# davrempe/humor

Hardware: AMD Instinct MI355X
Metric: fitting closure evaluations/s (stage-3 objective fwd+bwd), batch=32 seq=60 per GPU (higher is better)
Workload: dtype f32

## Files before the change

### humor_amd/_lib.py

```python
import ctypes as C
import os

_HERE = os.path.dirname(os.path.abspath(__file__))
DEFAULT_LIB = os.path.join(_HERE, 'csrc', 'libhumor_amd.so')

HA_OK = 0
ABI_VERSION = 7

c_float_p = C.POINTER(C.c_float)
c_int_p = C.POINTER(C.c_int32)


class MlpDesc(C.Structure):
    _fields_ = [('n_linear', C.c_int), ('in_dim', C.c_int), ('skip_dim', C.c_int), ('out_dims', C.c_int * 8),
                ('w', C.c_void_p * 8), ('b', C.c_void_p * 8), ('gn_gamma', C.c_void_p * 8), ('gn_beta', C.c_void_p * 8)]


FIT_NTERMS = 17


class GmmArgs(C.Structure):
    _fields_ = ([('B', C.c_int), ('K', C.c_int), ('D', C.c_int), ('nseg', C.c_int), ('seg', C.c_void_p * 4), ('seg_width', C.c_int * 4),
                 ('seg_stride', C.c_int * 4)] + [(n, C.c_void_p) for n in ('means', 'Linv', 'LinvT', 'cst', 'lp', 'gpart', 'nll', 'g_x')])

# ... 49 lines not shown
    'ha_device_arch': (C.c_int, [C.c_int, C.c_char_p, C.c_int]),
    'ha_tune_set': (C.c_int, [C.c_char_p, C.c_int]),
    'ha_debug_cu_poison': (C.c_int, [C.c_uint, C.POINTER(C.c_uint), C.c_void_p]),
    'ha_smpl_model_create': (C.c_int, [C.POINTER(C.c_void_p), C.c_int, C.c_int, C.c_int, C.c_int] + [C.c_void_p] * 6),
    'ha_smpl_model_destroy': (C.c_int, [C.c_void_p]),
    'ha_smpl_model_info': (C.c_int, [C.c_void_p, C.c_int, C.POINTER(C.c_int)]),
    'ha_smpl_model_define_subset': (C.c_int, [C.c_void_p, C.c_int, C.c_void_p, C.c_int]),
    'ha_smpl_forward': (C.c_int, [C.c_void_p, C.c_int, C.c_int, C.c_int] + [C.c_void_p] * 8 + [C.c_int, C.c_void_p]),
    'ha_smpl_workspace': (C.c_int, [C.c_void_p, C.c_int, C.c_int, C.POINTER(C.c_int64), C.POINTER(C.c_int64)]),
    'ha_smpl_backward': (C.c_int, [C.c_void_p, C.c_int, C.c_int, C.c_int] + [C.c_void_p] * 7 + [C.c_void_p]),
    'ha_smpl_forward_split': (C.c_int, [C.c_void_p, C.c_int, C.c_int, C.c_int] + [C.c_void_p] * 3 + [C.c_int] + [C.c_void_p] * 3),
    'ha_smpl_backward_split': (C.c_int, [C.c_void_p, C.c_int, C.c_int, C.c_int] + [C.c_void_p] * 2 + [C.c_int] + [C.c_void_p] * 6),
    'ha_smpl_forward_parts': (C.c_int, [C.c_void_p, C.c_int, C.c_int, C.c_int] + [C.c_void_p] * 3 + [C.c_int, C.c_void_p, C.c_int] + [C.c_void_p] * 3),
    'ha_smpl_backward_parts': (C.c_int, [C.c_void_p, C.c_int, C.c_int, C.c_int] + [C.c_void_p] * 3 + [C.c_int, C.c_int, C.c_void_p, C.c_int, C.c_int]
                               + [C.c_void_p] * 10),
    'ha_seq_sum_add': (C.c_int, [C.c_int, C.c_int, C.c_int] + [C.c_void_p] * 5),
    'ha_humor_rollout_backward_ex': (C.c_int, [C.c_void_p, C.c_int, C.c_int] + [C.c_void_p] * 8 + [C.c_void_p]),
    'ha_smpl_backward_dense_workspace': (C.c_int, [C.c_void_p, C.c_int, C.c_int, C.POINTER(C.c_int64)]),
    'ha_smpl_backward_dense': (C.c_int, [C.c_void_p, C.c_int, C.c_int] + [C.c_void_p] * 10 + [C.c_void_p]),
    'ha_lbs_skin': (C.c_int, [C.c_void_p, C.c_int] + [C.c_void_p] * 4 + [C.c_void_p]),
    'ha_rodrigues_fwd': (C.c_int, [C.c_int, C.c_void_p, C.c_void_p, C.c_void_p]),
    'ha_rodrigues_bwd': (C.c_int, [C.c_int, C.c_void_p, C.c_void_p, C.c_void_p, C.c_void_p]),
    'ha_rotmat_to_aa_fwd': (C.c_int, [C.c_int, C.c_void_p, C.c_void_p, C.c_void_p]),
    'ha_rotmat_to_aa_bwd': (C.c_int, [C.c_int, C.c_void_p, C.c_void_p, C.c_void_p, C.c_void_p]),
    'ha_rot6d_to_rotmat_fwd': (C.c_int, [C.c_int, C.c_void_p, C.c_void_p, C.c_void_p]),
    'ha_rot6d_to_rotmat_bwd': (C.c_int, [C.c_int, C.c_void_p, C.c_void_p, C.c_void_p, C.c_void_p]),
    'ha_rot9d_to_rotmat_fwd': (C.c_int, [C.c_int, C.c_void_p, C.c_void_p, C.c_void_p]),
    'ha_rot9d_to_rotmat_bwd': (C.c_int, [C.c_int, C.c_void_p, C.c_void_p, C.c_void_p, C.c_void_p]),
    'ha_humor_net_create': (C.c_int, [C.POINTER(C.c_void_p), C.c_int, C.POINTER(MlpDesc), C.POINTER(MlpDesc)]),
    'ha_humor_net_destroy': (C.c_int, [C.c_void_p]),
# ... 111 lines not shown
```

### humor_amd/csrc/smpl.hip

```cpp
#include <stdarg.h>
#include <string.h>
#include <algorithm>

#include <vector>

#include "smpl_model.h"
#ifndef HA_SIMT_EMU
#include "lane_reduce.h"
#endif

namespace ha {

static thread_local char g_err[512] = "";
void set_error(const char* fmt, ...) {
  va_list ap;
  va_start(ap, fmt);
  vsnprintf(g_err, sizeof(g_err), fmt, ap);
  va_end(ap);
}

}

namespace ha {
int g_skin_variant = -1;
int g_dense_gA_sparse = 2;
int g_dense_bwd_waves = 0;
extern int g_layer_finish, g_gemm_rm, g_rollout_groups, g_gemm_ks, g_gemm_fold, g_rollout_persist, g_rollout_persist_bwd, g_rollout_persist_inject, g_rollout_pipe, g_rollout_pipe_bwd;
extern unsigned g_cu_poison;
extern int g_loss_merge;
}
extern "C" int ha_tune_set(const char* key, int value) {
  HA_REQUIRE(key, "ha_tune_set: null key");
  if (strcmp(key, "skin_variant") == 0) { ha::g_skin_variant = value; return HA_OK; }
  if (strcmp(key, "dense_bwd_waves") == 0) { ha::g_dense_bwd_waves = value; return HA_OK; }
  if (strcmp(key, "dense_gA_sparse") == 0) { ha::g_dense_gA_sparse = value; return HA_OK; }
  if (strcmp(key, "layer_finish") == 0) { ha::g_layer_finish = value; return HA_OK; }
  if (strcmp(key, "gemm_rm") == 0) { ha::g_gemm_rm = value; return HA_OK; }
  if (strcmp(key, "rollout_groups") == 0) { ha::g_rollout_groups = value; return HA_OK; }
  if (strcmp(key, "gemm_ks") == 0) { ha::g_gemm_ks = value; return HA_OK; }
  if (strcmp(key, "gemm_fold") == 0) { ha::g_gemm_fold = value; return HA_OK; }
  if (strcmp(key, "rollout_persist") == 0) { ha::g_rollout_persist = value; return HA_OK; }
  if (strcmp(key, "rollout_persist_bwd") == 0) { ha::g_rollout_persist_bwd = value; return HA_OK; }
  if (strcmp(key, "rollout_pipe") == 0) { ha::g_rollout_pipe = value; return HA_OK; }
  if (strcmp(key, "rollout_pipe_bwd") == 0) { ha::g_rollout_pipe_bwd = value; return HA_OK; }
  if (strcmp(key, "loss_merge") == 0) { ha::g_loss_merge = value; return HA_OK; }
  if (strcmp(key, "rollout_persist_inject") == 0) { ha::g_rollout_persist_inject = value; return HA_OK; }
  if (strcmp(key, "cu_poison") == 0) { ha::g_cu_poison = (unsigned)value; return HA_OK; }
  ha::set_error("ha_tune_set: unknown key '%s'", key);
  return HA_ERR_INVALID_ARG;
}
extern "C" const char* ha_last_error(void) { return ha::g_err; }
extern "C" int ha_abi_version(void) { return 7; }
extern "C" int ha_device_arch(int device, char* buf, int buflen) {
  HA_REQUIRE(buf && buflen > 0, "ha_device_arch: null buffer");
  hipDeviceProp_t prop;
  HA_CHECK_HIP(hipGetDeviceProperties(&prop, device));
  snprintf(buf, buflen, "%s", prop.gcnArchName);
  return HA_OK;
}

namespace ha {

template <typename T>
static int upload(T** dst, const std::vector<T>& src) {
  *dst = nullptr;
  if (src.empty()) return HA_OK;
  HA_CHECK_HIP(hipMalloc((void**)dst, src.size() * sizeof(T)));
// ... 290 lines not shown
  const float* Jt; const float* Js; const int32_t* parents; const int32_t* jdepth;
  const int32_t* child_start; const int32_t* child_idx; const int32_t* anc; int nrounds;
  int J, NB, Kfull, Kfull_pad, kf4, depth;
  const float* Pd_v; const float* Pd_k; int Kp; const float* w; const int32_t* idx; const float* Wc;
  int nverts, nchunks, nnz;
  int N, n_active, Kc;
  const float* pose; const float* betas; const float* transl;
  float* verts; float* joints; float* A_out; float* coeffT; int Npad;
  int n_head, jstride;
  const float* g_verts; const float* g_joints;
  float* g_pose; float* g_betas; float* g_transl;
  const float* gA_in; const float* gco_part; int gco_ks, gco_rows, gco_ld; const float* gtl_part; int gtl_np;
  const float* pose_body; int betas_div; int gj_rows, gj_stride;
  float* g_body;
  const float* add_root; const float* add_body; const float* add_betas; const float* add_transl;
};

__device__ __forceinline__ const float* pose_of(const FrameParams& p, int f, int j, int J) {
  if (!p.pose_body) return p.pose + ((size_t)f * J + j) * 3;
  return j == 0 ? p.pose + (size_t)f * 3 : p.pose_body + ((size_t)f * (p.n_active - 1) + (j - 1)) * 3;
}
__device__ __forceinline__ const float* betas_of(const FrameParams& p, int f) {
  return p.betas + (size_t)(p.betas_div > 1 ? f / p.betas_div : f) * p.NB;
}

constexpr int FW = 4;

__device__ __forceinline__ void wave_sum16_all(float (&v)[16]) {
#ifdef HA_SIMT_EMU
#pragma unroll
  for (int i = 0; i < 16; ++i) {
// ... 183 lines not shown
  float* coeff = smem + wave * per_wave;
  float* Gs = coeff + p.kf4;
  int f = blockIdx.x * FW + wave;
  const bool valid = f < p.N;
  if (!valid) f = p.N - 1;

  SPT(0, 0);
  JointState s;
  joint_forward(p, f, lane, coeff, Gs, s);
  SPT(0, 1);

  float tl[3] = {0.f, 0.f, 0.f};
  if (p.transl) { tl[0] = p.transl[(size_t)f * 3]; tl[1] = p.transl[(size_t)f * 3 + 1]; tl[2] = p.transl[(size_t)f * 3 + 2]; }

  const bool isj = lane < p.J;
  float A[12];
  if (isj) {
    float gj[3];
    mat3_vec(s.G, s.Jr, gj);
#pragma unroll
    for (int i = 0; i < 9; ++i) A[i] = s.G[i];
#pragma unroll
    for (int c = 0; c < 3; ++c) A[9 + c] = s.G[9 + c] - gj[c];
#pragma unroll
    for (int i = 0; i < 12; ++i) Gs[lane * 12 + i] = A[i];
    if (valid) {
      if (p.joints) {
#pragma unroll
        for (int c = 0; c < 3; ++c) p.joints[((size_t)f * p.jstride + lane) * 3 + c] = s.G[9 + c] + tl[c];
      }
// ... 11 lines not shown
      v.x = 4 * q < p.kf4 ? coeff[4 * q] : 0.f;
      v.y = 4 * q + 1 < p.kf4 ? coeff[4 * q + 1] : 0.f;
      v.z = 4 * q + 2 < p.kf4 ? coeff[4 * q + 2] : 0.f;
      v.w = 4 * q + 3 < p.kf4 ? coeff[4 * q + 3] : 0.f;
      *reinterpret_cast<float4*>(p.coeffT + ((size_t)q * p.Npad + f) * 4) = v;
    }
  }
  if (p.verts) {
    for (int chunk = 0; chunk < p.nchunks; ++chunk) {
      float vp[3], T[12];
      SkinEntries sk;
      load_skin(p, chunk, lane, sk);
      SPT(0, 2);
      blend_vertex_block(p, chunk, wave, lane, smem, per_wave, smem + FW * per_wave, vp);
      SPT(0, 3);
      blend_transform(p, chunk, lane, sk, Gs, T);
      const int v = chunk * 64 + lane;
      if (valid && v < p.nverts) {
        float o[3];
        mat3_vec(T, vp, o);
        float* dst = v < p.n_head ? p.joints + ((size_t)f * p.jstride + p.J + v) * 3
                                  : p.verts + ((size_t)f * (p.nverts - p.n_head) + (v - p.n_head)) * 3;
        dst[0] = o[0] + T[9] + tl[0];
        dst[1] = o[1] + T[10] + tl[1];
        dst[2] = o[2] + T[11] + tl[2];
      }
      if (chunk + 1 < p.nchunks) __syncthreads();
    }
  }
  SPT(0, 4);
// ... 16 lines not shown
  float* gvp = msg + bwd_msg_floats(J);
  float* gco = gvp + 192;
  int f = blockIdx.x * FW + wave;
  const bool valid = f < p.N;
  if (!valid) f = p.N - 1;
  const bool isj = lane < J;

  constexpr int kChildReg = 5;
  int ch_reg[kChildReg], ch_c0 = 0, ch_c1 = 0;
  if (isj) { ch_c0 = p.child_start[lane]; ch_c1 = p.child_start[lane + 1]; }
#pragma unroll
  for (int u = 0; u < kChildReg; ++u) ch_reg[u] = ch_c0 + u < ch_c1 ? p.child_idx[ch_c0 + u] : -1;

  SPT(1, 0);
  JointState s;
  joint_forward(p, f, lane, coeff, Gs, s);
  SPT(1, 1);
  if (isj) {
    float gj[3];
    mat3_vec(s.G, s.Jr, gj);
#pragma unroll
    for (int i = 0; i < 9; ++i) As[lane * 12 + i] = s.G[i];
#pragma unroll
    for (int c = 0; c < 3; ++c) As[lane * 12 + 9 + c] = s.G[9 + c] - gj[c];
  }
  __syncthreads();

  float gco_reg[kMaxKM];
#pragma unroll
  for (int m = 0; m < kMaxKM; ++m) gco_reg[m] = 0.f;
  const int off_gvp = p.kf4 + J * 24 + bwd_msg_floats(J), off_gco = off_gvp + 192;
// ... 7 lines not shown
#pragma unroll
  for (int i = 0; i < 12; ++i) gAr[i] = 0.f;
  if (p.g_verts || (p.n_head > 0 && p.g_joints)) {
    for (int chunk = 0; chunk < p.nchunks; ++chunk) {
      float vp[3], T[12];
      SkinEntries sk;
      load_skin(p, chunk, lane, sk);
      const int v = chunk * 64 + lane;
      float g[3] = {0.f, 0.f, 0.f};
      if (v < p.nverts) {
        const float* src = v < p.n_head ? ((p.g_joints && (p.gj_rows == 0 || J + v < p.gj_rows)) ? p.g_joints + ((size_t)f * (p.gj_stride ? p.gj_stride : p.jstride) + J + v) * 3 : nullptr)
                                        : (p.g_verts ? p.g_verts + ((size_t)f * (p.nverts - p.n_head) + (v - p.n_head)) * 3 : nullptr);
        if (src) { g[0] = src[0]; g[1] = src[1]; g[2] = src[2]; }
      }
      SPT(1, 2);
      blend_vertex_block(p, chunk, wave, lane, smem, per_wave, smem + FW * per_wave, vp);
      SPT(1, 3);
      blend_transform(p, chunk, lane, sk, As, T);
      gtl[0] += g[0]; gtl[1] += g[1]; gtl[2] += g[2];
      float gv[3];
      mat3_tvec(T, g, gv);
      gvp[lane] = gv[0]; gvp[64 + lane] = gv[1]; gvp[128 + lane] = gv[2];
      {
        float u[12];
#pragma unroll
        for (int a = 0; a < 3; ++a) {
          u[a * 3 + 0] = g[a] * vp[0]; u[a * 3 + 1] = g[a] * vp[1]; u[a * 3 + 2] = g[a] * vp[2];
          u[9 + a] = g[a];
        }
        lds_st12(msg + lane * 12, u);
        wave_sync();
// ... 1090 lines not shown
  HA_REQUIRE(n_head >= 0 && n_head <= m->sets[slot].n, "ha_smpl_backward_split: n_head=%d out of range 0..%d", n_head, m->sets[slot].n);
  DeviceGuard guard(m->device);
  FrameParams p;
  fill_model(p, m, slot);
  p.N = N; p.n_active = n_active; p.Kc = m->NB + 1 + (n_active - 1) * 9;
  p.pose = pose; p.betas = betas;
  p.g_verts = g_verts_tail; p.g_joints = g_joints_ext;
  p.g_pose = g_pose; p.g_betas = g_betas; p.g_transl = g_transl;
  p.n_head = n_head; p.jstride = m->J + n_head;
  const size_t lds = ((size_t)FW * bwd_wave_floats((m->Kfull_pad + 3) & ~3, m->J) + kXchFloats) * sizeof(float);
  HA_LAUNCH(smpl_frame_bwd_kernel, dim3(ceil_div(N, FW)), dim3(FW * 64), lds, (hipStream_t)stream, p);
  HA_LAUNCH_CHECK();
  return HA_OK;
}

extern "C" int ha_smpl_forward_parts(const ha_smpl_model* m, int slot, int N, int n_active, const float* root, const float* body,
                                     const float* betas, int betas_div, const float* transl, int n_head, float* joints_ext,
                                     float* verts_tail, void* stream) {
  int rc = check_common("ha_smpl_forward_parts", m, slot, N, n_active);
  if (rc != HA_OK) return rc;
  HA_REQUIRE(root && betas && joints_ext && (body || n_active == 1), "ha_smpl_forward_parts: root, body, betas and joints_ext are required");
  HA_REQUIRE(betas_div >= 1 && N % betas_div == 0, "ha_smpl_forward_parts: betas_div=%d must divide N=%d", betas_div, N);
  HA_REQUIRE(n_head >= 0 && n_head <= m->sets[slot].n, "ha_smpl_forward_parts: n_head=%d out of range 0..%d", n_head, m->sets[slot].n);
  const bool joints_only = !verts_tail && n_head == 0;
  HA_REQUIRE(verts_tail || n_head == m->sets[slot].n || joints_only, "ha_smpl_forward_parts: verts_tail is required for the vertices behind the head");
  DeviceGuard guard(m->device);
  FrameParams p;
  fill_model(p, m, slot);
  if (joints_only) { p.nverts = 0; p.nchunks = 0; }
  p.N = N; p.n_active = n_active; p.Kc = m->NB + 1 + (n_active - 1) * 9;
  p.pose = root; p.pose_body = body ? body : root; p.betas = betas; p.betas_div = betas_div; p.transl = transl;
  p.joints = joints_ext; p.verts = verts_tail ? verts_tail : joints_ext;
  p.n_head = n_head; p.jstride = m->J + n_head;
  const size_t lds = ((size_t)FW * (((m->Kfull_pad + 3) & ~3) + m->J * 12) + kXchFloats) * sizeof(float);
  HA_LAUNCH(smpl_frame_fwd_kernel, dim3(ceil_div(N, FW)), dim3(FW * 64), lds, (hipStream_t)stream, p);
  HA_LAUNCH_CHECK();
  return HA_OK;
}

extern "C" int ha_smpl_backward_parts(const ha_smpl_model* m, int slot, int N, int n_active, const float* root, const float* body,
                                      const float* betas, int betas_div, int n_head, const float* g_joints_ext, int gj_rows,
                                      int gj_stride, const float* g_verts_tail, const float* add_root, const float* add_body,
                                      const float* add_betas, const float* add_transl, float* g_root, float* g_body, float* g_betas,
                                      float* g_transl, void* stream) {
  int rc = check_common("ha_smpl_backward_parts", m, slot, N, n_active);
  if (rc != HA_OK) return rc;
  HA_REQUIRE(root && betas && g_root && (body || n_active == 1), "ha_smpl_backward_parts: root, body, betas and g_root are required");
  HA_REQUIRE(betas_div >= 1 && N % betas_div == 0, "ha_smpl_backward_parts: betas_div=%d must divide N=%d", betas_div, N);
  HA_REQUIRE(n_head >= 0 && n_head <= m->sets[slot].n, "ha_smpl_backward_parts: n_head=%d out of range 0..%d", n_head, m->sets[slot].n);
  HA_REQUIRE(gj_rows >= 0 && gj_rows <= m->J + n_head && gj_stride >= 0, "ha_smpl_backward_parts: gj_rows=%d out of range", gj_rows);
  DeviceGuard guard(m->device);
  FrameParams p;
  fill_model(p, m, slot);
  p.N = N; p.n_active = n_active; p.Kc = m->NB + 1 + (n_active - 1) * 9;
  p.pose = root; p.pose_body = body ? body : root; p.betas = betas; p.betas_div = betas_div;
  if (!g_verts_tail && (n_head == 0 || !g_joints_ext || (gj_rows != 0 && gj_rows <= m->J))) { p.nverts = 0; p.nchunks = 0; }
  p.g_verts = g_verts_tail; p.g_joints = g_joints_ext; p.gj_rows = gj_rows; p.gj_stride = gj_stride;
  p.g_pose = g_root; p.g_body = g_body; p.g_betas = g_betas; p.g_transl = g_transl;
  p.add_root = add_root; p.add_body = add_body; p.add_betas = add_betas; p.add_transl = add_transl;
  p.n_head = n_head; p.jstride = m->J + n_head;
  const size_t lds = ((size_t)FW * bwd_wave_floats((m->Kfull_pad + 3) & ~3, m->J) + kXchFloats) * sizeof(float);
  HA_LAUNCH(smpl_frame_bwd_kernel, dim3(ceil_div(N, FW)), dim3(FW * 64), lds, (hipStream_t)stream, p);
  HA_LAUNCH_CHECK();
  return HA_OK;
}

namespace ha {
__global__ __launch_bounds__(256) void seq_sum_add_kernel(const float* __restrict__ src, const float* __restrict__ add1,
                                                          const float* __restrict__ add2, float* __restrict__ out, int T, int W) {
  extern __shared__ __attribute__((aligned(16))) float smem[];
  seq_sum_add_block(src, add1, add2, out, blockIdx.x, T, W, smem);
}
}

extern "C" int ha_seq_sum_add(int B, int T, int W, const float* src, const float* add1, const float* add2, float* out, void* stream) {
  HA_REQUIRE(src && out && B >= 1 && T >= 1 && W >= 1 && W <= 64, "ha_seq_sum_add: need src, out, B, T >= 1 and 1 <= W <= 64");
  HA_LAUNCH(seq_sum_add_kernel, dim3(B), dim3(256), 256 * sizeof(float), (hipStream_t)stream, src, add1, add2, out, T, W);
  HA_LAUNCH_CHECK();
  return HA_OK;
// ... 82 lines not shown
```

### humor_amd/stage3.py

```python
import ctypes as C

import torch

from . import _lib


def _new(dev, *sh):
    return torch.empty(sh, dtype=torch.float32, device=dev)


def _out(cfg, name, dev, *shape):
    t = cfg.get('grad_out', {}).get(name) if cfg.get('grad_out') else None
    if t is not None and tuple(t.shape) == tuple(shape) and t.is_contiguous() and t.dtype == torch.float32 and t.device == dev:
        return t
    return _new(dev, *shape)


def _c(x):
    if x is None or (x.dtype is torch.float32 and x.is_contiguous()):
        return x
    return x.detach().contiguous().float()


def _p(x):
    return _lib.ptr(x) if x is not None else None


def _sum_opt(a, b):
    if a is None:
        return b
    if b is None:
        return a
    return a + b


class Stage3Head(torch.autograd.Function):

    @staticmethod
    def forward(ctx, cfg, latent_pose, trans, root_orient, betas, floor, trans_vel, joints_vel, root_orient_vel):
        lib, sm, vp = cfg['lib'], cfg['smpl'], cfg['vposer']
# ... 1 lines not shown
        z, tr, ro, be, fl, tv, jv, rv = ins
        B, dev = z.shape[0], z.device
        st = _lib.stream_ptr(z)
        nws = cfg.setdefault('_vposer_ws', {}).get(B)
        if nws is None:
            n = C.c_int64()
            lib.call('ha_mlp_workspace', vp.ptr, B, C.byref(n))
            nws = cfg['_vposer_ws'][B] = n.value
        vws = _new(dev, nws)
        pose0 = _new(dev, B, vp.out_dim // 2)
        lib.call('ha_mlp_forward', vp.ptr, B, _p(z), 1, _p(pose0), _p(vws), st)
        h = sm['handle']
        slot, n_head, tail = sm['slot_all'], 0, None
        jrows = sm['J']
        joints = _new(dev, B, jrows, 3)
        lib.call('ha_smpl_forward_parts', h.ptr, slot, B, sm['n_active'], _p(ro), _p(pose0), _p(be), 1, _p(tr), n_head, _p(joints), _p(tail), st)
        out = dict(past_in=_new(dev, B, 339), trans_p=_new(dev, B, 3), root_p=_new(dev, B, 3), joints_p=_new(dev, B, 22, 3),
                   c2p_R=_new(dev, B, 3, 3), c2p_t=_new(dev, B, 3), root_height=_new(dev, B, 1))
        a = _lib.FitPreArgs()
        a.B = B
        for k, v in dict(floor=fl, trans0=tr, root0=ro, pose0=pose0, jcam=joints, trans_vel=tv, joints_vel=jv, root_orient_vel=rv, **out).items():
            setattr(a, k, v.data_ptr())
        a.jcam_stride = jrows * 3
        lib.call('ha_fit_pre_forward', C.byref(a), st)
        ctx.cfg, ctx.vws, ctx.slot, ctx.n_head, ctx.jrows = cfg, vws, slot, n_head, jrows
        ctx.save_for_backward(z, tr, ro, be, fl, tv, jv, rv, pose0, joints)
        ctx.set_materialize_grads(False)
        return (pose0, out['past_in'], out['trans_p'], out['root_p'], out['joints_p'], out['c2p_R'], out['c2p_t'], out['root_height'],
                floor, trans_vel, joints_vel, root_orient_vel, betas)

    @staticmethod
    def backward(ctx, g_pose0, g_past_in, g_trans_p, g_root_p, g_joints_p, g_c2p_R, g_c2p_t, g_root_height, g_floor_t, g_tv_t, g_jv_t,
                 g_rv_t, g_betas_t):
        cfg = ctx.cfg
        lib, sm, vp = cfg['lib'], cfg['smpl'], cfg['vposer']
        z, tr, ro, be, fl, tv, jv, rv, pose0, joints = ctx.saved_tensors
        B, dev = z.shape[0], z.device
        st = _lib.stream_ptr(z)
        keep = [_c(g) for g in (g_pose0, g_past_in, g_trans_p, g_root_p, g_joints_p, g_c2p_R, g_c2p_t, g_root_height, g_floor_t, g_tv_t,
                                g_jv_t, g_rv_t, g_betas_t)]
# ... 2 lines not shown
                 g_trans_vel=_out(cfg, 'trans_vel', dev, B, 3), g_joints_vel=_out(cfg, 'joints_vel', dev, B, 22, 3),
                 g_root_orient_vel=_out(cfg, 'root_orient_vel', dev, B, 3))
        a = _lib.FitPreArgs()
        a.B = B
        fields = dict(floor=fl, trans0=tr, root0=ro, pose0=pose0, jcam=joints, trans_vel=tv, joints_vel=jv, root_orient_vel=rv,
                      g_past_in=g_past_in, g_trans_p=g_trans_p, g_root_p=g_root_p, g_joints_p=g_joints_p, g_c2p_R=g_c2p_R, g_c2p_t=g_c2p_t,
                      g_root_height=g_root_height, add_floor=g_floor_t, add_pose0=g_pose0, add_trans_vel=g_tv_t, add_joints_vel=g_jv_t,
                      add_root_orient_vel=g_rv_t, **o)
        for k, v in fields.items():
            if v is not None:
                setattr(a, k, v.data_ptr())
        a.jcam_stride = ctx.jrows * 3
        lib.call('ha_fit_pre_backward', C.byref(a), st)
        g_root, g_body = _out(cfg, 'root_orient', dev, B, 3), _new(dev, B, 63)
        g_betas, g_transl = _out(cfg, 'betas', dev, B, be.shape[1]), _out(cfg, 'trans', dev, B, 3)
        lib.call('ha_smpl_backward_parts', sm['handle'].ptr, ctx.slot, B, sm['n_active'], _p(ro), _p(pose0), _p(be), 1, ctx.n_head,
                 _p(o['g_jcam']), 22, 22, None, _p(o['g_root0']), _p(o['g_pose0']), _p(g_betas_t), _p(o['g_trans0']),
                 _p(g_root), _p(g_body), _p(g_betas), _p(g_transl), st)
        g_z = _out(cfg, 'latent_pose', dev, B, vp.in_dim)
        lib.call('ha_mlp_backward', vp.ptr, B, _p(g_body), 1, _p(ctx.vws), _p(g_z), st)
        return None, g_z, g_transl, g_root, g_betas, o['g_floor'], o['g_trans_vel'], o['g_joints_vel'], o['g_root_orient_vel']


class Stage3Body(torch.autograd.Function):

    @staticmethod
    def forward(ctx, cfg, world, trans0, root0, pose0, joints0, c2p_R, c2p_t, betas):
        lib, sm = cfg['lib'], cfg['smpl']
        world, trans0, root0, pose0, joints0, c2p_R, c2p_t, be = (_c(x) for x in (world, trans0, root0, pose0, joints0, c2p_R, c2p_t, betas))
        B, S = world.shape[0], world.shape[1]
        T, dev = S + 1, world.device
        N = B * T
        st = _lib.stream_ptr(world)
        cam = c2p_R is not None
        post = dict(trans=_new(dev, B, T, 3), root_orient=_new(dev, B, T, 3), pose_body=_new(dev, B, T, 63), joints=_new(dev, B, T, 22, 3),
                    contacts_conf=_new(dev, B, T, 22), contacts=_new(dev, B, T, 22))
        if cam:
            post.update(cam_trans=_new(dev, B, T, 3), cam_root_orient=_new(dev, B, T, 3))
        a = _lib.RolloutPostArgs()
        a.B, a.S = B, S
        for k, v in dict(world=world, trans0=trans0, root0=root0, pose0=pose0, joints0=joints0, c2p_R=c2p_R, c2p_t=c2p_t, **post).items():
            if v is not None:
                setattr(a, k, v.data_ptr())
        lib.call('ha_rollout_post_forward', C.byref(a), st)
        h, n_sel = sm['handle'], sm['n_sel']
        jx, nv = sm['J'] + n_sel, sm['n_all'] - n_sel
        jtr, verts = _new(dev, B, T, jx, 3), _new(dev, B, T, nv, 3)
        lib.call('ha_smpl_forward_parts', h.ptr, sm['slot_all'], N, sm['n_active'], _p(post['root_orient']), _p(post['pose_body']), _p(be), T,
                 _p(post['trans']), n_sel, _p(jtr), _p(verts) if nv > 0 else None, st)
        cam_jtr = cam_verts = None
        if cam:
            cam_jtr, cam_verts = torch.empty_like(jtr), torch.empty_like(verts)
            r = _lib.RigidImageArgs()
            r.N, r.J, r.V = N, jx, nv
            for k, v in dict(joints=jtr, verts=verts, root=post['root_orient'], trans=post['trans'], root2=post['cam_root_orient'],
                             trans2=post['cam_trans'], joints2=cam_jtr, verts2=cam_verts).items():
                if v.numel():
                    setattr(r, k, v.data_ptr())
            lib.call('ha_rigid_image_forward', C.byref(r), st)
        ctx.cfg, ctx.cam, ctx.dims = cfg, cam, (B, S, jx, nv)
        ctx.save_for_backward(world, trans0, root0, c2p_R, c2p_t, be, post['trans'], post['root_orient'], post['pose_body'], post['contacts_conf'],
                              post.get('cam_trans'), post.get('cam_root_orient'), jtr, verts)
        ctx.set_materialize_grads(False)
        ctx.mark_non_differentiable(post['contacts'])
        return (jtr, verts, cam_jtr, cam_verts, post['trans'], post['root_orient'], post['pose_body'], post['joints'], post['contacts_conf'],
                post['contacts'], post.get('cam_trans'), post.get('cam_root_orient'), betas)

    @staticmethod
    def backward(ctx, g_jtr, g_verts, g_cam_jtr, g_cam_verts, g_trans, g_root, g_pose, g_ro_joints, g_conf, _g_lab, g_ct, g_cr, g_betas_t):
        cfg = ctx.cfg
        lib, sm = cfg['lib'], cfg['smpl']
        world, trans0, root0, c2p_R, c2p_t, be, trans, root_orient, pose_body, conf, cam_trans, cam_root, jtr, verts = ctx.saved_tensors
        B, S, jx, nv = ctx.dims
        T, dev = S + 1, world.device
        N = B * T
# ... 4 lines not shown
        if ctx.cam and (g_cam_jtr is not None or g_cam_verts is not None):
            o = dict(g_joints=torch.empty_like(jtr), g_verts=torch.empty_like(verts), g_root=_new(dev, N, 3), g_trans=_new(dev, N, 3),
                     g_root2=_new(dev, N, 3), g_trans2=_new(dev, N, 3))
            r = _lib.RigidImageArgs()
            r.N, r.J, r.V = N, jx, nv
            for k, v in dict(joints=jtr, verts=verts, root=root_orient, trans=trans, root2=cam_root, trans2=cam_trans, g_joints2=g_cam_jtr,
                             g_verts2=g_cam_verts, g_joints_add=g_jtr, g_verts_add=g_verts, **o).items():
                if v is not None and v.numel():
                    setattr(r, k, v.data_ptr())
            lib.call('ha_rigid_image_backward', C.byref(r), st)
            g_jtr, g_verts = o['g_joints'], (o['g_verts'] if nv > 0 else None)
            add_root, add_transl = _sum_opt(g_root, o['g_root']), _sum_opt(g_trans, o['g_trans'])
            g_t2, g_r2 = _sum_opt(g_ct, o['g_trans2']), _sum_opt(g_cr, o['g_root2'])
        NB = be.shape[1]
        g_ro, g_pb, g_bf, g_tl = _new(dev, B, T, 3), _new(dev, B, T, 63), _new(dev, N, NB), _new(dev, B, T, 3)
        lib.call('ha_smpl_backward_parts', sm['handle'].ptr, sm['slot_all'], N, sm['n_active'], _p(root_orient), _p(pose_body), _p(be), T,
                 sm['n_sel'], _p(g_jtr), 0, 0, _p(g_verts), _p(add_root), _p(g_pose), None, _p(add_transl),
                 _p(g_ro), _p(g_pb), _p(g_bf), _p(g_tl), st)
        g_betas = _new(dev, B, NB)
        gw, gt0, gr0, gp0, gj0 = _new(dev, B, S, 348), _new(dev, B, 3), _new(dev, B, 3), _new(dev, B, 63), _new(dev, B, 22, 3)
        gR, gt = (_new(dev, B, 3, 3), _new(dev, B, 3)) if ctx.cam else (None, None)
        partial = _new(dev, N, 15)
        a = _lib.RolloutPostArgs()
        a.B, a.S = B, S
        fields = dict(world=world, trans0=trans0, root0=root0, c2p_R=c2p_R, c2p_t=c2p_t, root_orient=root_orient, contacts_conf=conf,
                      g_trans=g_tl, g_root_orient=g_ro, g_pose_body=g_pb, g_joints=g_ro_joints, g_contacts_conf=g_conf,
                      g_cam_trans=g_t2, g_cam_root_orient=g_r2, g_world=gw, g_trans0=gt0, g_root0=gr0, g_pose0=gp0, g_joints0=gj0,
                      g_c2p_R=gR, g_c2p_t=gt, partial=partial, sum_src=g_bf, sum_add1=g_betas_t, sum_out=g_betas)
        for k, v in fields.items():
            if v is not None:
                setattr(a, k, v.data_ptr())
        a.sum_W = NB
        lib.call('ha_rollout_post_backward', C.byref(a), st)
# ... 2 lines not shown
```

### include/humor_amd.h

```cpp
#ifndef HUMOR_AMD_H
#define HUMOR_AMD_H

#include <stdint.h>

#ifdef __cplusplus
extern "C" {
#endif

#define HA_OK 0
#define HA_ERR_INVALID_ARG 1
#define HA_ERR_HIP 2
#define HA_ERR_UNSUPPORTED 3

const char* ha_last_error(void);
int ha_abi_version(void);
int ha_device_arch(int device, char* buf, int buflen);
int ha_tune_set(const char* key, int value);
int ha_debug_cu_poison(unsigned int pattern, unsigned int* surviving_words, void* stream);

typedef struct ha_smpl_model ha_smpl_model;

int ha_smpl_model_create(ha_smpl_model** out, int device, int V, int J, int NB,
                         const float* v_template, const float* shapedirs, const float* posedirs,
                         const float* J_regressor, const float* weights, const int32_t* parents);
// ... 15 lines not shown
                     float* g_pose, float* g_betas, float* g_transl, void* stream);

int ha_smpl_forward_split(const ha_smpl_model* m, int slot, int N, int n_active, const float* pose, const float* betas,
                          const float* transl, int n_head, float* joints_ext, float* verts_tail, void* stream);
int ha_smpl_backward_split(const ha_smpl_model* m, int slot, int N, int n_active, const float* pose, const float* betas,
                           int n_head, const float* g_joints_ext, const float* g_verts_tail, float* g_pose, float* g_betas,
                           float* g_transl, void* stream);

int ha_smpl_forward_parts(const ha_smpl_model* m, int slot, int N, int n_active, const float* root, const float* body,
                          const float* betas, int betas_div, const float* transl, int n_head, float* joints_ext, float* verts_tail,
                          void* stream);
int ha_smpl_backward_parts(const ha_smpl_model* m, int slot, int N, int n_active, const float* root, const float* body,
                           const float* betas, int betas_div, int n_head, const float* g_joints_ext, int gj_rows, int gj_stride,
                           const float* g_verts_tail, const float* add_root, const float* add_body, const float* add_betas,
                           const float* add_transl, float* g_root, float* g_body, float* g_betas, float* g_transl, void* stream);
int ha_seq_sum_add(int B, int T, int W, const float* src, const float* add1, const float* add2, float* out, void* stream);

int ha_smpl_backward_dense_workspace(const ha_smpl_model* m, int N, int n_active_joints, int64_t* ws_floats);
int ha_smpl_backward_dense(const ha_smpl_model* m, int N, int n_active_joints, const float* pose, const float* betas,
                           const float* g_verts, const float* g_joints, const float* v_posed, const float* A, float* ws,
                           float* g_pose, float* g_betas, float* g_transl, void* stream);

int ha_lbs_skin(const ha_smpl_model* m, int N, const float* v_posed, const float* A, const float* transl,
                float* verts, void* stream);

int ha_rodrigues_fwd(int n, const float* aa , float* R , void* stream);
int ha_rodrigues_bwd(int n, const float* aa, const float* gR , float* g_aa , void* stream);
int ha_rotmat_to_aa_fwd(int n, const float* R , float* aa , void* stream);
int ha_rotmat_to_aa_bwd(int n, const float* R, const float* g_aa, float* gR, void* stream);
int ha_rot6d_to_rotmat_fwd(int n, const float* x , float* R , void* stream);
// ... 197 lines not shown
```

Measured before the change: 651.5.

## Stash SMPL joint transforms and posed vertices in forward for reuse in backward

The SMPL frame forward kernel now writes each joint's global transform and rest joint position, plus the blended posed vertices per chunk, into a device stash buffer. The backward kernel reads these values instead of re-running joint_forward and blend_vertex_block, so the recomputation of the kinematic chain and the blend-shape GEMV in backward goes away. The cost is extra global memory writes in forward, a stash allocation per call, and extra reads in backward. The stage-3 Python paths now call the new stash entry points, and a tune key can disable the stash.

New measurement: 656.1 (median of 6 runs). About the same (+0.7%).

```diff
diff --git a/humor_amd/_lib.py b/humor_amd/_lib.py
--- a/humor_amd/_lib.py
+++ b/humor_amd/_lib.py
@@ -5,7 +5,7 @@
 DEFAULT_LIB = os.path.join(_HERE, 'csrc', 'libhumor_amd.so')
 
 HA_OK = 0
-ABI_VERSION = 7
+ABI_VERSION = 8
 
 c_float_p = C.POINTER(C.c_float)
 c_int_p = C.POINTER(C.c_int32)
@@ -87,6 +87,11 @@
     'ha_smpl_forward_parts': (C.c_int, [C.c_void_p, C.c_int, C.c_int, C.c_int] + [C.c_void_p] * 3 + [C.c_int, C.c_void_p, C.c_int] + [C.c_void_p] * 3),
     'ha_smpl_backward_parts': (C.c_int, [C.c_void_p, C.c_int, C.c_int, C.c_int] + [C.c_void_p] * 3 + [C.c_int, C.c_int, C.c_void_p, C.c_int, C.c_int]
                                + [C.c_void_p] * 10),
+    'ha_smpl_parts_stash_floats': (C.c_int, [C.c_void_p, C.c_int, C.c_int, C.c_int, C.POINTER(C.c_int64)]),
+    'ha_smpl_forward_parts_stash': (C.c_int, [C.c_void_p, C.c_int, C.c_int, C.c_int] + [C.c_void_p] * 3 + [C.c_int, C.c_void_p, C.c_int] + [C.c_void_p] * 3
+                                    + [C.c_int64, C.c_void_p]),
+    'ha_smpl_backward_parts_stash': (C.c_int, [C.c_void_p, C.c_int, C.c_int, C.c_int] + [C.c_void_p] * 3 + [C.c_int, C.c_int, C.c_void_p, C.c_int, C.c_int]
+                                     + [C.c_void_p] * 10 + [C.c_int64, C.c_void_p]),
     'ha_seq_sum_add': (C.c_int, [C.c_int, C.c_int, C.c_int] + [C.c_void_p] * 5),
     'ha_humor_rollout_backward_ex': (C.c_int, [C.c_void_p, C.c_int, C.c_int] + [C.c_void_p] * 8 + [C.c_void_p]),
     'ha_smpl_backward_dense_workspace': (C.c_int, [C.c_void_p, C.c_int, C.c_int, C.POINTER(C.c_int64)]),
diff --git a/humor_amd/csrc/smpl.hip b/humor_amd/csrc/smpl.hip
--- a/humor_amd/csrc/smpl.hip
+++ b/humor_amd/csrc/smpl.hip
@@ -28,6 +28,7 @@
 extern int g_layer_finish, g_gemm_rm, g_rollout_groups, g_gemm_ks, g_gemm_fold, g_rollout_persist, g_rollout_persist_bwd, g_rollout_persist_inject, g_rollout_pipe, g_rollout_pipe_bwd;
 extern unsigned g_cu_poison;
 extern int g_loss_merge;
+int g_smpl_stash = 1;
 }
 extern "C" int ha_tune_set(const char* key, int value) {
   HA_REQUIRE(key, "ha_tune_set: null key");
@@ -44,13 +45,14 @@
   if (strcmp(key, "rollout_pipe") == 0) { ha::g_rollout_pipe = value; return HA_OK; }
   if (strcmp(key, "rollout_pipe_bwd") == 0) { ha::g_rollout_pipe_bwd = value; return HA_OK; }
   if (strcmp(key, "loss_merge") == 0) { ha::g_loss_merge = value; return HA_OK; }
+  if (strcmp(key, "smpl_stash") == 0) { ha::g_smpl_stash = value; return HA_OK; }
   if (strcmp(key, "rollout_persist_inject") == 0) { ha::g_rollout_persist_inject = value; return HA_OK; }
   if (strcmp(key, "cu_poison") == 0) { ha::g_cu_poison = (unsigned)value; return HA_OK; }
   ha::set_error("ha_tune_set: unknown key '%s'", key);
   return HA_ERR_INVALID_ARG;
 }
 extern "C" const char* ha_last_error(void) { return ha::g_err; }
-extern "C" int ha_abi_version(void) { return 7; }
+extern "C" int ha_abi_version(void) { return 8; }
 extern "C" int ha_device_arch(int device, char* buf, int buflen) {
   HA_REQUIRE(buf && buflen > 0, "ha_device_arch: null buffer");
   hipDeviceProp_t prop;
@@ -371,7 +373,10 @@
   const float* pose_body; int betas_div; int gj_rows, gj_stride;
   float* g_body;
   const float* add_root; const float* add_body; const float* add_betas; const float* add_transl;
+  float* stash_w; const float* stash_r;
 };
+
+__host__ __device__ inline size_t stash_joint_floats(int N, int J) { return (size_t)N * J * 16; }
 
 __device__ __forceinline__ const float* pose_of(const FrameParams& p, int f, int j, int J) {
   if (!p.pose_body) return p.pose + ((size_t)f * J + j) * 3;
@@ -585,6 +590,13 @@
   if (p.transl) { tl[0] = p.transl[(size_t)f * 3]; tl[1] = p.transl[(size_t)f * 3 + 1]; tl[2] = p.transl[(size_t)f * 3 + 2]; }
 
   const bool isj = lane < p.J;
+  if (p.stash_w && valid && isj) {
+    float4* q = reinterpret_cast<float4*>(p.stash_w) + (size_t)f * 4 * p.J + lane;
+    q[0] = make_float4(s.G[0], s.G[1], s.G[2], s.G[3]);
+    q[p.J] = make_float4(s.G[4], s.G[5], s.G[6], s.G[7]);
+    q[2 * p.J] = make_float4(s.G[8], s.G[9], s.G[10], s.G[11]);
+    q[3 * p.J] = make_float4(s.Jr[0], s.Jr[1], s.Jr[2], 0.f);
+  }
   float A[12];
   if (isj) {
     float gj[3];
@@ -626,6 +638,10 @@
       SPT(0, 2);
       blend_vertex_block(p, chunk, wave, lane, smem, per_wave, smem + FW * per_wave, vp);
       SPT(0, 3);
+      if (p.stash_w && valid) {
+        float* q = p.stash_w + stash_joint_floats(p.N, p.J) + ((size_t)f * p.nchunks + chunk) * 192 + lane;
+        q[0] = vp[0]; q[64] = vp[1]; q[128] = vp[2];
+      }
       blend_transform(p, chunk, lane, sk, Gs, T);
       const int v = chunk * 64 + lane;
       if (valid && v < p.nverts) {
@@ -672,7 +688,25 @@
 
   SPT(1, 0);
   JointState s;
-  joint_forward(p, f, lane, coeff, Gs, s);
+  if (p.stash_r) {
+#pragma unroll
+    for (int i = 0; i < 12; ++i) s.G[i] = 0.f;
+    s.Jr[0] = s.Jr[1] = s.Jr[2] = 0.f;
+    s.parent = -1;
+    s.depth = -1;
+    if (isj) {
+      const float4* q = reinterpret_cast<const float4*>(p.stash_r) + (size_t)f * 4 * J + lane;
+      const float4 a = q[0], b = q[J], c = q[2 * J], d = q[3 * J];
+      s.parent = p.parents[lane];
+      s.depth = p.jdepth[lane];
+      s.G[0] = a.x; s.G[1] = a.y; s.G[2] = a.z; s.G[3] = a.w; s.G[4] = b.x; s.G[5] = b.y; s.G[6] = b.z; s.G[7] = b.w;
+      s.G[8] = c.x; s.G[9] = c.y; s.G[10] = c.z; s.G[11] = c.w;
+      s.Jr[0] = d.x; s.Jr[1] = d.y; s.Jr[2] = d.z;
+      lds_st12(Gs + lane * 12, s.G);
+    }
+  } else {
+    joint_forward(p, f, lane, coeff, Gs, s);
+  }
   SPT(1, 1);
   if (isj) {
     float gj[3];
@@ -710,7 +744,12 @@
         if (src) { g[0] = src[0]; g[1] = src[1]; g[2] = src[2]; }
       }
       SPT(1, 2);
-      blend_vertex_block(p, chunk, wave, lane, smem, per_wave, smem + FW * per_wave, vp);
+      if (p.stash_r) {
+        const float* q = p.stash_r + stash_joint_floats(p.N, J) + ((size_t)f * p.nchunks + chunk) * 192 + lane;
+        vp[0] = q[0]; vp[1] = q[64]; vp[2] = q[128];
+      } else {
+        blend_vertex_block(p, chunk, wave, lane, smem, per_wave, smem + FW * per_wave, vp);
+      }
       SPT(1, 3);
       blend_transform(p, chunk, lane, sk, As, T);
       gtl[0] += g[0]; gtl[1] += g[1]; gtl[2] += g[2];
@@ -1831,20 +1870,46 @@
   return HA_OK;
 }
 
-extern "C" int ha_smpl_forward_parts(const ha_smpl_model* m, int slot, int N, int n_active, const float* root, const float* body,
-                                     const float* betas, int betas_div, const float* transl, int n_head, float* joints_ext,
-                                     float* verts_tail, void* stream) {
-  int rc = check_common("ha_smpl_forward_parts", m, slot, N, n_active);
+namespace ha {
+static int64_t parts_stash_floats(const ha_smpl_model* m, int slot, int N, bool with_vertices) {
+  return (int64_t)stash_joint_floats(N, m->J) + (with_vertices ? (int64_t)N * m->sets[slot].nchunks * 192 : 0);
+}
+static int check_stash(const char* fn, const ha_smpl_model* m, int slot, int N, bool with_vertices, const void* stash, int64_t stash_floats) {
+  HA_REQUIRE(stash && (reinterpret_cast<uintptr_t>(stash) & 15) == 0, "%s: the stash must be a 16-byte aligned device buffer", fn);
+  const int64_t want = parts_stash_floats(m, slot, N, with_vertices);
+  HA_REQUIRE(stash_floats == want, "%s: stash_floats=%lld, but ha_smpl_parts_stash_floats gives %lld for slot %d, N=%d, %s", fn,
+             (long long)stash_floats, (long long)want, slot, N, with_vertices ? "with vertices" : "joints only");
+  return HA_OK;
+}
+}
+
+extern "C" int ha_smpl_parts_stash_floats(const ha_smpl_model* m, int slot, int N, int with_vertices, int64_t* floats) {
+  int rc = check_common("ha_smpl_parts_stash_floats", m, slot, N, 1);
   if (rc != HA_OK) return rc;
-  HA_REQUIRE(root && betas && joints_ext && (body || n_active == 1), "ha_smpl_forward_parts: root, body, betas and joints_ext are required");
-  HA_REQUIRE(betas_div >= 1 && N % betas_div == 0, "ha_smpl_forward_parts: betas_div=%d must divide N=%d", betas_div, N);
-  HA_REQUIRE(n_head >= 0 && n_head <= m->sets[slot].n, "ha_smpl_forward_parts: n_head=%d out of range 0..%d", n_head, m->sets[slot].n);
+  HA_REQUIRE(floats, "ha_smpl_parts_stash_floats: null argument");
+  *floats = parts_stash_floats(m, slot, N, with_vertices != 0);
+  return HA_OK;
+}
+
+static int smpl_forward_parts(const char* fn, const ha_smpl_model* m, int slot, int N, int n_active, const float* root, const float* body,
+                              const float* betas, int betas_div, const float* transl, int n_head, float* joints_ext, float* verts_tail,
+                              bool stashing, float* stash, int64_t stash_floats, void* stream) {
+  int rc = check_common(fn, m, slot, N, n_active);
+  if (rc != HA_OK) return rc;
+  HA_REQUIRE(root && betas && joints_ext && (body || n_active == 1), "%s: root, body, betas and joints_ext are required", fn);
+  HA_REQUIRE(betas_div >= 1 && N % betas_div == 0, "%s: betas_div=%d must divide N=%d", fn, betas_div, N);
+  HA_REQUIRE(n_head >= 0 && n_head <= m->sets[slot].n, "%s: n_head=%d out of range 0..%d", fn, n_head, m->sets[slot].n);
   const bool joints_only = !verts_tail && n_head == 0;
-  HA_REQUIRE(verts_tail || n_head == m->sets[slot].n || joints_only, "ha_smpl_forward_parts: verts_tail is required for the vertices behind the head");
+  HA_REQUIRE(verts_tail || n_head == m->sets[slot].n || joints_only, "%s: verts_tail is required for the vertices behind the head", fn);
   DeviceGuard guard(m->device);
   FrameParams p;
   fill_model(p, m, slot);
   if (joints_only) { p.nverts = 0; p.nchunks = 0; }
+  if (stashing) {
+    rc = check_stash(fn, m, slot, N, !joints_only, stash, stash_floats);
+    if (rc != HA_OK) return rc;
+    if (g_smpl_stash) p.stash_w = stash;
+  }
   p.N = N; p.n_active = n_active; p.Kc = m->NB + 1 + (n_active - 1) * 9;
   p.pose = root; p.pose_body = body ? body : root; p.betas = betas; p.betas_div = betas_div; p.transl = transl;
   p.joints = joints_ext; p.verts = verts_tail ? verts_tail : joints_ext;
@@ -1855,23 +1920,42 @@
   return HA_OK;
 }
 
-extern "C" int ha_smpl_backward_parts(const ha_smpl_model* m, int slot, int N, int n_active, const float* root, const float* body,
-                                      const float* betas, int betas_div, int n_head, const float* g_joints_ext, int gj_rows,
-                                      int gj_stride, const float* g_verts_tail, const float* add_root, const float* add_body,
-                                      const float* add_betas, const float* add_transl, float* g_root, float* g_body, float* g_betas,
-                                      float* g_transl, void* stream) {
-  int rc = check_common("ha_smpl_backward_parts", m, slot, N, n_active);
+extern "C" int ha_smpl_forward_parts(const ha_smpl_model* m, int slot, int N, int n_active, const float* root, const float* body,
+                                     const float* betas, int betas_div, const float* transl, int n_head, float* joints_ext,
+                                     float* verts_tail, void* stream) {
+  return smpl_forward_parts("ha_smpl_forward_parts", m, slot, N, n_active, root, body, betas, betas_div, transl, n_head, joints_ext, verts_tail,
+                            false, nullptr, 0, stream);
+}
+
+extern "C" int ha_smpl_forward_parts_stash(const ha_smpl_model* m, int slot, int N, int n_active, const float* root, const float* body,
+                                           const float* betas, int betas_div, const float* transl, int n_head, float* joints_ext,
+                                           float* verts_tail, float* stash, int64_t stash_floats, void* stream) {
+  return smpl_forward_parts("ha_smpl_forward_parts_stash", m, slot, N, n_active, root, body, betas, betas_div, transl, n_head, joints_ext,
+                            verts_tail, true, stash, stash_floats, stream);
+}
+
+static int smpl_backward_parts(const char* fn, const ha_smpl_model* m, int slot, int N, int n_active, const float* root, const float* body,
+                               const float* betas, int betas_div, int n_head, const float* g_joints_ext, int gj_rows, int gj_stride,
+                               const float* g_verts_tail, const float* add_root, const float* add_body, const float* add_betas,
+                               const float* add_transl, float* g_root, float* g_body, float* g_betas, float* g_transl, bool stashed,
+                               const float* stash, int64_t stash_floats, void* stream) {
+  int rc = check_common(fn, m, slot, N, n_active);
   if (rc != HA_OK) return rc;
-  HA_REQUIRE(root && betas && g_root && (body || n_active == 1), "ha_smpl_backward_parts: root, body, betas and g_root are required");
-  HA_REQUIRE(betas_div >= 1 && N % betas_div == 0, "ha_smpl_backward_parts: betas_div=%d must divide N=%d", betas_div, N);
-  HA_REQUIRE(n_head >= 0 && n_head <= m->sets[slot].n, "ha_smpl_backward_parts: n_head=%d out of range 0..%d", n_head, m->sets[slot].n);
-  HA_REQUIRE(gj_rows >= 0 && gj_rows <= m->J + n_head && gj_stride >= 0, "ha_smpl_backward_parts: gj_rows=%d out of range", gj_rows);
+  HA_REQUIRE(root && betas && g_root && (body || n_active == 1), "%s: root, body, betas and g_root are required", fn);
+  HA_REQUIRE(betas_div >= 1 && N % betas_div == 0, "%s: betas_div=%d must divide N=%d", fn, betas_div, N);
+  HA_REQUIRE(n_head >= 0 && n_head <= m->sets[slot].n, "%s: n_head=%d out of range 0..%d", fn, n_head, m->sets[slot].n);
+  HA_REQUIRE(gj_rows >= 0 && gj_rows <= m->J + n_head && gj_stride >= 0, "%s: gj_rows=%d out of range", fn, gj_rows);
   DeviceGuard guard(m->device);
   FrameParams p;
   fill_model(p, m, slot);
   p.N = N; p.n_active = n_active; p.Kc = m->NB + 1 + (n_active - 1) * 9;
   p.pose = root; p.pose_body = body ? body : root; p.betas = betas; p.betas_div = betas_div;
   if (!g_verts_tail && (n_head == 0 || !g_joints_ext || (gj_rows != 0 && gj_rows <= m->J))) { p.nverts = 0; p.nchunks = 0; }
+  if (stashed) {
+    rc = check_stash(fn, m, slot, N, p.nchunks > 0, stash, stash_floats);
+    if (rc != HA_OK) return rc;
+    if (g_smpl_stash) p.stash_r = stash;
+  }
   p.g_verts = g_verts_tail; p.g_joints = g_joints_ext; p.gj_rows = gj_rows; p.gj_stride = gj_stride;
   p.g_pose = g_root; p.g_body = g_body; p.g_betas = g_betas; p.g_transl = g_transl;
   p.add_root = add_root; p.add_body = add_body; p.add_betas = add_betas; p.add_transl = add_transl;
@@ -1880,6 +1964,25 @@
   HA_LAUNCH(smpl_frame_bwd_kernel, dim3(ceil_div(N, FW)), dim3(FW * 64), lds, (hipStream_t)stream, p);
   HA_LAUNCH_CHECK();
   return HA_OK;
+}
+
+extern "C" int ha_smpl_backward_parts(const ha_smpl_model* m, int slot, int N, int n_active, const float* root, const float* body,
+                                      const float* betas, int betas_div, int n_head, const float* g_joints_ext, int gj_rows,
+                                      int gj_stride, const float* g_verts_tail, const float* add_root, const float* add_body,
+                                      const float* add_betas, const float* add_transl, float* g_root, float* g_body, float* g_betas,
+                                      float* g_transl, void* stream) {
+  return smpl_backward_parts("ha_smpl_backward_parts", m, slot, N, n_active, root, body, betas, betas_div, n_head, g_joints_ext, gj_rows, gj_stride,
+                             g_verts_tail, add_root, add_body, add_betas, add_transl, g_root, g_body, g_betas, g_transl, false, nullptr, 0, stream);
+}
+
+extern "C" int ha_smpl_backward_parts_stash(const ha_smpl_model* m, int slot, int N, int n_active, const float* root, const float* body,
+                                            const float* betas, int betas_div, int n_head, const float* g_joints_ext, int gj_rows,
+                                            int gj_stride, const float* g_verts_tail, const float* add_root, const float* add_body,
+                                            const float* add_betas, const float* add_transl, float* g_root, float* g_body, float* g_betas,
+                                            float* g_transl, const float* stash, int64_t stash_floats, void* stream) {
+  return smpl_backward_parts("ha_smpl_backward_parts_stash", m, slot, N, n_active, root, body, betas, betas_div, n_head, g_joints_ext, gj_rows,
+                             gj_stride, g_verts_tail, add_root, add_body, add_betas, add_transl, g_root, g_body, g_betas, g_transl, true, stash,
+                             stash_floats, stream);
 }
 
 namespace ha {
diff --git a/humor_amd/stage3.py b/humor_amd/stage3.py
--- a/humor_amd/stage3.py
+++ b/humor_amd/stage3.py
@@ -24,6 +24,16 @@
 
 def _p(x):
     return _lib.ptr(x) if x is not None else None
+
+
+def _stash_floats(cfg, slot, N, with_vertices):
+    sizes = cfg.setdefault('_smpl_stash', {})
+    n = sizes.get((slot, N, with_vertices))
+    if n is None:
+        v = C.c_int64()
+        cfg['lib'].call('ha_smpl_parts_stash_floats', cfg['smpl']['handle'].ptr, slot, N, int(with_vertices), C.byref(v))
+        n = sizes[(slot, N, with_vertices)] = v.value
+    return n
 
 
 def _sum_opt(a, b):
@@ -55,7 +65,9 @@
         slot, n_head, tail = sm['slot_all'], 0, None
         jrows = sm['J']
         joints = _new(dev, B, jrows, 3)
-        lib.call('ha_smpl_forward_parts', h.ptr, slot, B, sm['n_active'], _p(ro), _p(pose0), _p(be), 1, _p(tr), n_head, _p(joints), _p(tail), st)
+        stash = _new(dev, _stash_floats(cfg, slot, B, False))
+        lib.call('ha_smpl_forward_parts_stash', h.ptr, slot, B, sm['n_active'], _p(ro), _p(pose0), _p(be), 1, _p(tr), n_head, _p(joints), _p(tail),
+                 _p(stash), stash.numel(), st)
         out = dict(past_in=_new(dev, B, 339), trans_p=_new(dev, B, 3), root_p=_new(dev, B, 3), joints_p=_new(dev, B, 22, 3),
                    c2p_R=_new(dev, B, 3, 3), c2p_t=_new(dev, B, 3), root_height=_new(dev, B, 1))
         a = _lib.FitPreArgs()
@@ -64,7 +76,7 @@
             setattr(a, k, v.data_ptr())
         a.jcam_stride = jrows * 3
         lib.call('ha_fit_pre_forward', C.byref(a), st)
-        ctx.cfg, ctx.vws, ctx.slot, ctx.n_head, ctx.jrows = cfg, vws, slot, n_head, jrows
+        ctx.cfg, ctx.vws, ctx.slot, ctx.n_head, ctx.jrows, ctx.stash = cfg, vws, slot, n_head, jrows, stash
         ctx.save_for_backward(z, tr, ro, be, fl, tv, jv, rv, pose0, joints)
         ctx.set_materialize_grads(False)
         return (pose0, out['past_in'], out['trans_p'], out['root_p'], out['joints_p'], out['c2p_R'], out['c2p_t'], out['root_height'],
@@ -97,9 +109,9 @@
         lib.call('ha_fit_pre_backward', C.byref(a), st)
         g_root, g_body = _out(cfg, 'root_orient', dev, B, 3), _new(dev, B, 63)
         g_betas, g_transl = _out(cfg, 'betas', dev, B, be.shape[1]), _out(cfg, 'trans', dev, B, 3)
-        lib.call('ha_smpl_backward_parts', sm['handle'].ptr, ctx.slot, B, sm['n_active'], _p(ro), _p(pose0), _p(be), 1, ctx.n_head,
+        lib.call('ha_smpl_backward_parts_stash', sm['handle'].ptr, ctx.slot, B, sm['n_active'], _p(ro), _p(pose0), _p(be), 1, ctx.n_head,
                  _p(o['g_jcam']), 22, 22, None, _p(o['g_root0']), _p(o['g_pose0']), _p(g_betas_t), _p(o['g_trans0']),
-                 _p(g_root), _p(g_body), _p(g_betas), _p(g_transl), st)
+                 _p(g_root), _p(g_body), _p(g_betas), _p(g_transl), _p(ctx.stash), ctx.stash.numel(), st)
         g_z = _out(cfg, 'latent_pose', dev, B, vp.in_dim)
         lib.call('ha_mlp_backward', vp.ptr, B, _p(g_body), 1, _p(ctx.vws), _p(g_z), st)
         return None, g_z, g_transl, g_root, g_betas, o['g_floor'], o['g_trans_vel'], o['g_joints_vel'], o['g_root_orient_vel']
@@ -129,8 +141,9 @@
         h, n_sel = sm['handle'], sm['n_sel']
         jx, nv = sm['J'] + n_sel, sm['n_all'] - n_sel
         jtr, verts = _new(dev, B, T, jx, 3), _new(dev, B, T, nv, 3)
-        lib.call('ha_smpl_forward_parts', h.ptr, sm['slot_all'], N, sm['n_active'], _p(post['root_orient']), _p(post['pose_body']), _p(be), T,
-                 _p(post['trans']), n_sel, _p(jtr), _p(verts) if nv > 0 else None, st)
+        stash = _new(dev, _stash_floats(cfg, sm['slot_all'], N, n_sel > 0 or nv > 0))
+        lib.call('ha_smpl_forward_parts_stash', h.ptr, sm['slot_all'], N, sm['n_active'], _p(post['root_orient']), _p(post['pose_body']), _p(be), T,
+                 _p(post['trans']), n_sel, _p(jtr), _p(verts) if nv > 0 else None, _p(stash), stash.numel(), st)
         cam_jtr = cam_verts = None
         if cam:
             cam_jtr, cam_verts = torch.empty_like(jtr), torch.empty_like(verts)
@@ -141,7 +154,7 @@
                 if v.numel():
                     setattr(r, k, v.data_ptr())
             lib.call('ha_rigid_image_forward', C.byref(r), st)
-        ctx.cfg, ctx.cam, ctx.dims = cfg, cam, (B, S, jx, nv)
+        ctx.cfg, ctx.cam, ctx.dims, ctx.stash = cfg, cam, (B, S, jx, nv), stash
         ctx.save_for_backward(world, trans0, root0, c2p_R, c2p_t, be, post['trans'], post['root_orient'], post['pose_body'], post['contacts_conf'],
                               post.get('cam_trans'), post.get('cam_root_orient'), jtr, verts)
         ctx.set_materialize_grads(False)
@@ -176,9 +189,10 @@
             g_t2, g_r2 = _sum_opt(g_ct, o['g_trans2']), _sum_opt(g_cr, o['g_root2'])
         NB = be.shape[1]
         g_ro, g_pb, g_bf, g_tl = _new(dev, B, T, 3), _new(dev, B, T, 63), _new(dev, N, NB), _new(dev, B, T, 3)
-        lib.call('ha_smpl_backward_parts', sm['handle'].ptr, sm['slot_all'], N, sm['n_active'], _p(root_orient), _p(pose_body), _p(be), T,
+        with_v = g_verts is not None or (sm['n_sel'] > 0 and g_jtr is not None)
+        lib.call('ha_smpl_backward_parts_stash', sm['handle'].ptr, sm['slot_all'], N, sm['n_active'], _p(root_orient), _p(pose_body), _p(be), T,
                  sm['n_sel'], _p(g_jtr), 0, 0, _p(g_verts), _p(add_root), _p(g_pose), None, _p(add_transl),
-                 _p(g_ro), _p(g_pb), _p(g_bf), _p(g_tl), st)
+                 _p(g_ro), _p(g_pb), _p(g_bf), _p(g_tl), _p(ctx.stash), _stash_floats(cfg, sm['slot_all'], N, with_v), st)
         g_betas = _new(dev, B, NB)
         gw, gt0, gr0, gp0, gj0 = _new(dev, B, S, 348), _new(dev, B, 3), _new(dev, B, 3), _new(dev, B, 63), _new(dev, B, 22, 3)
         gR, gt = (_new(dev, B, 3, 3), _new(dev, B, 3)) if ctx.cam else (None, None)
diff --git a/include/humor_amd.h b/include/humor_amd.h
--- a/include/humor_amd.h
+++ b/include/humor_amd.h
@@ -53,6 +53,15 @@
                            const float* betas, int betas_div, int n_head, const float* g_joints_ext, int gj_rows, int gj_stride,
                            const float* g_verts_tail, const float* add_root, const float* add_body, const float* add_betas,
                            const float* add_transl, float* g_root, float* g_body, float* g_betas, float* g_transl, void* stream);
+int ha_smpl_parts_stash_floats(const ha_smpl_model* m, int slot, int N, int with_vertices, int64_t* floats);
+int ha_smpl_forward_parts_stash(const ha_smpl_model* m, int slot, int N, int n_active, const float* root, const float* body,
+                                const float* betas, int betas_div, const float* transl, int n_head, float* joints_ext, float* verts_tail,
+                                float* stash, int64_t stash_floats, void* stream);
+int ha_smpl_backward_parts_stash(const ha_smpl_model* m, int slot, int N, int n_active, const float* root, const float* body,
+                                 const float* betas, int betas_div, int n_head, const float* g_joints_ext, int gj_rows, int gj_stride,
+                                 const float* g_verts_tail, const float* add_root, const float* add_body, const float* add_betas,
+                                 const float* add_transl, float* g_root, float* g_body, float* g_betas, float* g_transl,
+                                 const float* stash, int64_t stash_floats, void* stream);
 int ha_seq_sum_add(int B, int T, int W, const float* src, const float* add1, const float* add2, float* out, void* stream);
 
 int ha_smpl_backward_dense_workspace(const ha_smpl_model* m, int N, int n_active_joints, int64_t* ws_floats);
```
